# KyanChen/RSPrompter

Hardware: NVIDIA H100
Metric: images/sec (higher is better)
Workload: dtype bf16

## Files before the change

rsprompter_b200/csrc/attention.cu:

```cuda
#include <cstdlib>

#include "attention.h"
#include "sm90.cuh"

namespace rsp {

constexpr float LOG2E = 1.4426950408889634f;

__device__ __forceinline__ float fast_exp2(float x) {
  float y;
  asm("ex2.approx.ftz.f32 %0, %1;" : "=f"(y) : "f"(x));
  return y;
}
__device__ __forceinline__ uint32_t pack_f16x2(float lo, float hi) {
  __half2 v = __floats2half2_rn(lo, hi);
  return *reinterpret_cast<uint32_t*>(&v);
}
__device__ __forceinline__ uint32_t bf16x2_to_f16x2(uint32_t w) {
  return pack_f16x2(__uint_as_float(w << 16), __uint_as_float(w & 0xffff0000u));
}

template <int HD, int S>
struct AttCfg {
  static constexpr int T = S * S;
  static constexpr int BM = 128;
  static constexpr int BN = 64;
  static constexpr int NQT = (T + BM - 1) / BM;
  static constexpr int NKT = (T + BN - 1) / BN;
  static constexpr int NREL = 2 * S - 1;
  static constexpr int NTAB = NREL <= 32 ? 32 : (NREL <= 64 ? 64 : 128);
  static constexpr int TAIL = HD - 64;
  static constexpr int STAGES = 4;
  static constexpr int SP = S + 4;
  __host__ __device__ static constexpr int tile_bytes(int rows) { return rows * (128 + 2 * TAIL); }
  static constexpr int STAGE_BYTES = 2 * tile_bytes(BN);
  static constexpr int smem_bytes(int qbuf) {
    return qbuf * tile_bytes(BM) + STAGES * STAGE_BYTES + 2 * tile_bytes(NTAB) + 2 * BM * SP * 4 + 8 * 64 + 1024;
  }
  static constexpr int QBUF = smem_bytes(2) <= 227 * 1024 ? 2 : 1;
  static constexpr int Q_OFF = 0;
  static constexpr int KV_OFF = Q_OFF + QBUF * tile_bytes(BM);
  static constexpr int TAB_OFF = KV_OFF + STAGES * STAGE_BYTES;
  static constexpr int BIAS_OFF = TAB_OFF + 2 * tile_bytes(NTAB);
  static constexpr int BAR_OFF = BIAS_OFF + 2 * BM * SP * 4;
  static constexpr int SMEM_BYTES = smem_bytes(QBUF);
  static constexpr int REG_PRODUCER = 40, REG_CONSUMER = 232;
  static_assert(HD == 64 || HD == 80, "head dim");
  static_assert(NREL <= 128, "table rows");
  static_assert(SMEM_BYTES <= 227 * 1024, "shared memory");
};

struct AttDev {
  __nv_bfloat16* out;
  const int* out_row_map;
  int H;
  int D;
  int n_items;
  float scale2;
};

template <int N, int TAIL>
__device__ __forceinline__ void qk_wgmma(float (&acc)[N / 2], uint32_t qa, uint32_t qtail, uint32_t b, int b_rows) {
  acc_fence(acc);
  wgmma_fence();
#pragma unroll
  for (int k = 0; k < 4; ++k)
    Wgmma<N>::template ss<0>(acc, make_gdesc(qa + 32 * k, 16, 1024), make_gdesc(b + 32 * k, 16, 1024), k);
  if constexpr (TAIL > 0)
    Wgmma<N>::template ss<0>(acc, make_gdesc_sw32(qtail, 16, 256), make_gdesc_sw32(b + b_rows * 128, 16, 256), 1);
  wgmma_commit();
  wgmma_wait<0>();
  acc_fence(acc);
}

template <int TAIL>
__device__ __forceinline__ void load_tile(uint32_t dst, int rows, const CUtensorMap* m, const CUtensorMap* mt,
                                          uint32_t bar, int col, int row, int seq) {
  tma_load_3d(dst, m, bar, col, row, seq);
  if constexpr (TAIL > 0) tma_load_3d(dst + rows * 128, mt, bar, col + 64, row, seq);
}

template <int HD, int S>
__global__ void __launch_bounds__(384, 1)
vit_attention_kernel(const __grid_constant__ CUtensorMap tm_q, const __grid_constant__ CUtensorMap tm_q_t,
                     const __grid_constant__ CUtensorMap tm_kv, const __grid_constant__ CUtensorMap tm_kv_t,
                     const __grid_constant__ CUtensorMap tm_rh, const __grid_constant__ CUtensorMap tm_rh_t,
                     const __grid_constant__ CUtensorMap tm_rw, const __grid_constant__ CUtensorMap tm_rw_t,
                     const AttDev p) {
  using C = AttCfg<HD, S>;
  constexpr int T = C::T, BM = C::BM, BN = C::BN, NKT = C::NKT, SP = C::SP, STAGES = C::STAGES, TAIL = C::TAIL;
  constexpr int QBUF = C::QBUF;
  constexpr uint32_t TILE_KV = C::tile_bytes(BN), TILE_TAB = C::tile_bytes(C::NTAB);
  extern __shared__ __align__(1024) uint8_t smem_raw[];
  uint8_t* smem = smem_raw + ((1024u - (smem_u32(smem_raw) & 1023u)) & 1023u);
  const uint32_t sbase = smem_u32(smem);
  float* relh = reinterpret_cast<float*>(smem + C::BIAS_OFF);
  float* relw = relh + BM * SP;
  uint64_t* bar_tab = reinterpret_cast<uint64_t*>(smem + C::BAR_OFF);
  uint64_t* bar_q = bar_tab + 1;
  uint64_t* bar_qe = bar_q + QBUF;
  uint64_t* bar_k = bar_qe + QBUF;
  uint64_t* bar_v = bar_k + STAGES;
  uint64_t* bar_vc = bar_v + STAGES;
  uint64_t* bar_e = bar_vc + STAGES;

  const int warp = threadIdx.x >> 5, lane = threadIdx.x & 31;
  auto decode = [&](int item, int& q0, int& head, int& seq) {
    q0 = (item % C::NQT) * BM;
    item /= C::NQT;
    head = item % p.H;
    seq = item / p.H;
  };

  if (threadIdx.x == 0) {
    tma_prefetch_desc(&tm_q);
    tma_prefetch_desc(&tm_kv);
    mbar_init(smem_u32(bar_tab), 1);
    for (int b = 0; b < QBUF; ++b) {
      mbar_init(smem_u32(&bar_q[b]), 1);
      mbar_init(smem_u32(&bar_qe[b]), 8);
    }
    for (int s = 0; s < STAGES; ++s) {
      mbar_init(smem_u32(&bar_k[s]), 1);
      mbar_init(smem_u32(&bar_v[s]), 1);
      mbar_init(smem_u32(&bar_vc[s]), 3);
      mbar_init(smem_u32(&bar_e[s]), 8);
    }
    fence_barrier_init();
  }
  __syncthreads();

  if (warp < 4) {
    setmaxnreg_dec<C::REG_PRODUCER>();
    if (warp == 0) {
      if (lane == 0) {
        const uint32_t bq = smem_u32(bar_tab);
        mbar_expect_tx(bq, 2 * TILE_TAB);
        tma_load_2d(sbase + C::TAB_OFF, &tm_rh, bq, 0, 0);
        tma_load_2d(sbase + C::TAB_OFF + TILE_TAB, &tm_rw, bq, 0, 0);
        if constexpr (TAIL > 0) {
          tma_load_2d(sbase + C::TAB_OFF + C::NTAB * 128, &tm_rh_t, bq, 64, 0);
          tma_load_2d(sbase + C::TAB_OFF + TILE_TAB + C::NTAB * 128, &tm_rw_t, bq, 64, 0);
        }
        int g = 0;
#pragma unroll 1
        for (int item = blockIdx.x, it = 0; item < p.n_items; item += gridDim.x, ++it) {
          int q0, head, seq;
          decode(item, q0, head, seq);
          const int colq = head * HD, colk = p.D + colq, colv = 2 * p.D + colq;
          const int qb = it % QBUF;
          mbar_wait(smem_u32(&bar_qe[qb]), ((it / QBUF) & 1) ^ 1);
          mbar_expect_tx(smem_u32(&bar_q[qb]), C::tile_bytes(BM));
          load_tile<TAIL>(sbase + C::Q_OFF + qb * C::tile_bytes(BM), BM, &tm_q, &tm_q_t, smem_u32(&bar_q[qb]),
                          colq, q0, seq);
#pragma unroll 1
          for (int j = 0; j < NKT; ++j, ++g) {
            const int s = g % STAGES;
            mbar_wait(smem_u32(&bar_e[s]), ((g / STAGES) & 1) ^ 1);
            const uint32_t kb = sbase + C::KV_OFF + s * C::STAGE_BYTES;
            mbar_expect_tx(smem_u32(&bar_k[s]), TILE_KV);
            load_tile<TAIL>(kb, BN, &tm_kv, &tm_kv_t, smem_u32(&bar_k[s]), colk, j * BN, seq);
            mbar_expect_tx(smem_u32(&bar_v[s]), TILE_KV);
            load_tile<TAIL>(kb + TILE_KV, BN, &tm_kv, &tm_kv_t, smem_u32(&bar_v[s]), colv, j * BN, seq);
          }
        }
      }
    } else {
      const int t = threadIdx.x - 32;
      const int n_tiles = ((p.n_items - static_cast<int>(blockIdx.x) + gridDim.x - 1) / gridDim.x) * NKT;
#pragma unroll 1
      for (int g = 0; g < n_tiles; ++g) {
        const int s = g % STAGES;
        mbar_wait(smem_u32(&bar_v[s]), (g / STAGES) & 1);
        uint4* v = reinterpret_cast<uint4*>(smem + C::KV_OFF + s * C::STAGE_BYTES + TILE_KV);
#pragma unroll 2
        for (int i = t; i < static_cast<int>(TILE_KV / 16); i += 96) {
          uint4 w = v[i];
          w.x = bf16x2_to_f16x2(w.x);
          w.y = bf16x2_to_f16x2(w.y);
          w.z = bf16x2_to_f16x2(w.z);
          w.w = bf16x2_to_f16x2(w.w);
          v[i] = w;
        }
        fence_proxy_async_smem();
        __syncwarp();
        if (lane == 0) mbar_arrive(smem_u32(&bar_vc[s]));
      }
    }
    return;
  }

  setmaxnreg_inc<C::REG_CONSUMER>();
  const int wg = (warp >> 2) - 1;
  const int r0 = wg * 64 + (warp & 3) * 16 + (lane >> 2);
  const int cq = 2 * (lane & 3);
  constexpr bool REG_W = BN % S == 0;
  constexpr int CPS = REG_W ? S / 8 : 1;
  mbar_wait(smem_u32(bar_tab), 0);
  int g = 0;
#pragma unroll 1
  for (int item = blockIdx.x, it = 0; item < p.n_items; item += gridDim.x, ++it) {
    int q0, head, seq;
    decode(item, q0, head, seq);
    const int qb = it % QBUF;
    const uint32_t qbase = sbase + C::Q_OFF + qb * C::tile_bytes(BM);
    const uint32_t qa = qbase + wg * 64 * 128;
    const uint32_t qtail = qbase + BM * 128 + wg * 64 * 32;

    mbar_wait(smem_u32(&bar_q[qb]), (it / QBUF) & 1);
    named_bar_sync(1 + wg, 128);
#pragma unroll 1
    for (int tab = 0; tab < 2; ++tab) {
      float acc[C::NTAB / 2];
      qk_wgmma<C::NTAB, TAIL>(acc, qa, qtail, sbase + C::TAB_OFF + tab * TILE_TAB, C::NTAB);
      float* dst = tab ? relw : relh;
#pragma unroll
      for (int x = 0; x < C::NTAB / 2; ++x) {
        const int r = r0 + 8 * ((x >> 1) & 1);
        const int tq = q0 + r;
        const int qc = tab ? tq % S : tq / S;
        const int t = 8 * (x >> 2) + cq + (x & 1);
        const int k = qc + S - 1 - t;
        if (t < C::NREL && k >= 0 && k < S) dst[r * SP + k] = acc[x] * LOG2E;
      }
    }
    named_bar_sync(1 + wg, 128);

    float rw[2][2 * CPS];
    if constexpr (REG_W) {
#pragma unroll
      for (int i = 0; i < 2; ++i)
#pragma unroll
        for (int m = 0; m < 2 * CPS; ++m) rw[i][m] = relw[(r0 + 8 * i) * SP + 8 * (m >> 1) + cq + (m & 1)];
    }

    float om[32], ot[8];
#pragma unroll
    for (int y = 0; y < 32; ++y) om[y] = 0.f;
#pragma unroll
    for (int y = 0; y < 8; ++y) ot[y] = 0.f;
    float m_run[2] = {-INFINITY, -INFINITY}, l_run[2] = {0.f, 0.f};
    const float scale2 = p.scale2;

#pragma unroll(REG_W ? 1 : NKT)
    for (int j = 0; j < NKT; ++j, ++g) {
      const int s = g % STAGES;
      const uint32_t ph = (g / STAGES) & 1;
      const uint32_t kb = sbase + C::KV_OFF + s * C::STAGE_BYTES, vb = kb + TILE_KV;
      mbar_wait(smem_u32(&bar_k[s]), ph);
      float sc[BN / 2];
      qk_wgmma<BN, TAIL>(sc, qa, qtail, kb, BN);
      if (j == NKT - 1) {
        __syncwarp();
        if (lane == 0) mbar_arrive(smem_u32(&bar_qe[qb]));
      }

      float mx[2] = {-INFINITY, -INFINITY};
      if constexpr (REG_W) {
        constexpr int NB = BN / S;
        float bh[2][NB];
#pragma unroll
        for (int i = 0; i < 2; ++i)
#pragma unroll
          for (int b = 0; b < NB; ++b) bh[i][b] = relh[(r0 + 8 * i) * SP + j * NB + b];
#pragma unroll
        for (int x = 0; x < BN / 2; ++x) {
          const int i = (x >> 1) & 1;
          const float t = fmaf(sc[x], scale2, bh[i][(x >> 2) / CPS] + rw[i][((x >> 2) % CPS) * 2 + (x & 1)]);
          sc[x] = t;
          mx[i] = fmaxf(mx[i], t);
        }
      } else {
#pragma unroll
        for (int x = 0; x < BN / 2; ++x) {
          const int i = (x >> 1) & 1;
          const int key = j * BN + 8 * (x >> 2) + cq + (x & 1);
          float t = -INFINITY;
          if (T % BN == 0 || key < T) {
            const int kh = key / S, kw = key - kh * S;
            const int r = r0 + 8 * i;
            t = fmaf(sc[x], scale2, relh[r * SP + kh] + relw[r * SP + kw]);
          }
          sc[x] = t;
          mx[i] = fmaxf(mx[i], t);
        }
      }
      float alpha[2];
#pragma unroll
      for (int i = 0; i < 2; ++i) {
        mx[i] = fmaxf(mx[i], __shfl_xor_sync(0xffffffffu, mx[i], 1));
        mx[i] = fmaxf(mx[i], __shfl_xor_sync(0xffffffffu, mx[i], 2));
        const float m_new = fmaxf(m_run[i], mx[i]);
        alpha[i] = fast_exp2(m_run[i] - m_new);
        m_run[i] = m_new;
        l_run[i] *= alpha[i];
      }
#pragma unroll
      for (int y = 0; y < 32; ++y) om[y] *= alpha[(y >> 1) & 1];
#pragma unroll
      for (int y = 0; y < 8; ++y) ot[y] *= alpha[(y >> 1) & 1];
      uint32_t pa[BN / 16][4];
#pragma unroll
      for (int kk = 0; kk < BN / 16; ++kk) {
#pragma unroll
        for (int h = 0; h < 4; ++h) {
          const int x = 8 * kk + 2 * h, i = h & 1;
          const float p0 = fast_exp2(sc[x] - m_run[i]), p1 = fast_exp2(sc[x + 1] - m_run[i]);
          l_run[i] += p0 + p1;
          pa[kk][h] = pack_f16x2(p0, p1);
        }
      }
      mbar_wait(smem_u32(&bar_vc[s]), ph);
      acc_fence(om);
      acc_fence(ot);
      wgmma_fence();
#pragma unroll
      for (int kk = 0; kk < BN / 16; ++kk) {
        WgmmaRsF16<64>::rs(om, pa[kk], make_gdesc(vb + kk * 2048, BN * 128, 1024));
        if constexpr (TAIL > 0) WgmmaRsF16<16>::rs(ot, pa[kk], make_gdesc_sw32(vb + BN * 128 + kk * 512, 256, 256));
      }
      wgmma_commit();
      wgmma_wait<0>();
      acc_fence(om);
      acc_fence(ot);
      __syncwarp();
      if (lane == 0) mbar_arrive(smem_u32(&bar_e[s]));
    }

#pragma unroll
    for (int i = 0; i < 2; ++i) {
      float l = l_run[i];
      l += __shfl_xor_sync(0xffffffffu, l, 1);
      l += __shfl_xor_sync(0xffffffffu, l, 2);
      const float inv = 1.0f / l;
      const int tq = q0 + r0 + 8 * i;
      if (tq >= T) continue;
      int dst = seq * T + tq;
      if (p.out_row_map) dst = __ldg(p.out_row_map + dst);
      if (dst < 0) continue;
      __nv_bfloat16* orow = p.out + static_cast<size_t>(dst) * p.D + head * HD + cq;
#pragma unroll
      for (int nb = 0; nb < 8; ++nb)
        *reinterpret_cast<uint32_t*>(orow + nb * 8) = pack_bf16x2(om[4 * nb + 2 * i] * inv, om[4 * nb + 2 * i + 1] * inv);
      if constexpr (TAIL > 0) {
#pragma unroll
        for (int nb = 0; nb < 2; ++nb)
          *reinterpret_cast<uint32_t*>(orow + 64 + nb * 8) =
              pack_bf16x2(ot[4 * nb + 2 * i] * inv, ot[4 * nb + 2 * i + 1] * inv);
      }
    }
  }
}

template <int HD, int S>
static int launch_att(const AttentionArgs& a, cudaStream_t stream) {
  using C = AttCfg<HD, S>;
  RSP_CHECK_ARG((reinterpret_cast<uintptr_t>(a.qkv) & 15) == 0 && (reinterpret_cast<uintptr_t>(a.rel_h) & 15) == 0 &&
                (reinterpret_cast<uintptr_t>(a.rel_w) & 15) == 0 && (reinterpret_cast<uintptr_t>(a.out) & 3) == 0,
                "attention: qkv / tables must be 16-byte aligned");
  AttDev p;
  p.out = static_cast<__nv_bfloat16*>(a.out);
  p.out_row_map = a.out_row_map;
  p.H = a.H; p.D = a.H * HD;
  p.scale2 = (1.0f / sqrtf(static_cast<float>(HD))) * LOG2E;
  const uint64_t ld = 3ull * p.D;
  const uint64_t qdims[3] = {ld, static_cast<uint64_t>(C::T), static_cast<uint64_t>(a.n_seq)};
  const uint64_t qstr[2] = {ld * 2, ld * 2 * C::T};
  const uint64_t tdims[2] = {static_cast<uint64_t>(HD), static_cast<uint64_t>(C::NREL)};
  const uint64_t tstr[1] = {static_cast<uint64_t>(HD) * 2};
  const uint32_t qbox[3] = {64, C::BM, 1}, qbox_t[3] = {16, C::BM, 1};
  const uint32_t kvbox[3] = {64, C::BN, 1}, kvbox_t[3] = {16, C::BN, 1};
  const uint32_t tbox[2] = {64, static_cast<uint32_t>(C::NTAB)}, tbox_t[2] = {16, static_cast<uint32_t>(C::NTAB)};
  CUtensorMap tq, tkv, th, tw, tq_t, tkv_t, th_t, tw_t;
  RSP_TRY(make_tmap_swizzled(&tq, a.qkv, 3, qdims, qstr, qbox, 0, 128));
  RSP_TRY(make_tmap_swizzled(&tkv, a.qkv, 3, qdims, qstr, kvbox, 0, 128));
  RSP_TRY(make_tmap_swizzled(&th, a.rel_h, 2, tdims, tstr, tbox, 0, 128));
  RSP_TRY(make_tmap_swizzled(&tw, a.rel_w, 2, tdims, tstr, tbox, 0, 128));
  if (C::TAIL > 0) {
    RSP_TRY(make_tmap_swizzled(&tq_t, a.qkv, 3, qdims, qstr, qbox_t, 0, 32));
    RSP_TRY(make_tmap_swizzled(&tkv_t, a.qkv, 3, qdims, qstr, kvbox_t, 0, 32));
    RSP_TRY(make_tmap_swizzled(&th_t, a.rel_h, 2, tdims, tstr, tbox_t, 0, 32));
    RSP_TRY(make_tmap_swizzled(&tw_t, a.rel_w, 2, tdims, tstr, tbox_t, 0, 32));
  } else {
    tq_t = tq; tkv_t = tkv; th_t = th; tw_t = tw;
  }
  auto kern = vit_attention_kernel<HD, S>;
  static bool attr_set_dev[kMaxDevices] = {};
  bool& attr_set = attr_set_dev[current_device()];
  if (!attr_set) {
    RSP_CHECK_CUDA(cudaFuncSetAttribute(kern, cudaFuncAttributeMaxDynamicSharedMemorySize, C::SMEM_BYTES));
    attr_set = true;
  }
  const long long items = static_cast<long long>(a.n_seq) * a.H * C::NQT;
  RSP_CHECK_ARG(items > 0 && items < (1ll << 31), "attention: %lld query tiles", items);
  p.n_items = static_cast<int>(items);
  const int grid = static_cast<int>(items < num_sms() ? items : num_sms());
  kern<<<grid, 384, C::SMEM_BYTES, stream>>>(tq, tq_t, tkv, tkv_t, th, th_t, tw, tw_t, p);
  RSP_CHECK_LAUNCH();
  return RSP_OK;
}

int vit_attention(const AttentionArgs& a, cudaStream_t stream) {
  RSP_CHECK_ARG(a.qkv && a.rel_h && a.rel_w && a.out, "attention: null pointer");
  RSP_CHECK_ARG(a.T == a.S * a.S, "attention: T=%d is not S^2 (S=%d)", a.T, a.S);
  RSP_CHECK_ARG(a.n_seq > 0 && a.H > 0, "attention: bad n_seq/H");
  if (a.S != 14 && a.S != 32 && a.S != 64)
    return vit_attention_simt(a, stream);
  if (a.hd == 64) {
    if (a.S == 64) return launch_att<64, 64>(a, stream);
    if (a.S == 32) return launch_att<64, 32>(a, stream);
    return launch_att<64, 14>(a, stream);
  }
  if (a.hd == 80) {
    if (a.S == 64) return launch_att<80, 64>(a, stream);
    if (a.S == 32) return launch_att<80, 32>(a, stream);
    return launch_att<80, 14>(a, stream);
  }
  set_last_error("attention: head dim %d unsupported (64, 80)", a.hd);
  return RSP_ERR_UNSUPPORTED;
}

__global__ void vit_attention_simt_kernel(const __nv_bfloat16* __restrict__ qkv,
                                          const __nv_bfloat16* __restrict__ rel_h,
                                          const __nv_bfloat16* __restrict__ rel_w,
                                          __nv_bfloat16* __restrict__ out, int T, int S, int H,
                                          int hd, float scale, const int* __restrict__ out_row_map) {
  const int D = H * hd;
  const int tq = blockIdx.x * blockDim.x + threadIdx.x;
  const int head = blockIdx.y;
  const int seq = blockIdx.z;
  if (tq >= T) return;
  const int qh = tq / S, qw = tq % S;
  const __nv_bfloat16* qp = qkv + (static_cast<size_t>(seq) * T + tq) * 3 * D + head * hd;
  float q[128];
  for (int d = 0; d < hd; ++d) q[d] = __bfloat162float(qp[d]);
  float rh[128], rw[128];
  for (int k = 0; k < S; ++k) {
    float ah = 0.f, aw = 0.f;
    const __nv_bfloat16* th = rel_h + static_cast<size_t>(qh - k + S - 1) * hd;
    const __nv_bfloat16* tw = rel_w + static_cast<size_t>(qw - k + S - 1) * hd;
    for (int d = 0; d < hd; ++d) {
      ah += q[d] * __bfloat162float(th[d]);
      aw += q[d] * __bfloat162float(tw[d]);
    }
    rh[k] = ah; rw[k] = aw;
  }
  float m = -INFINITY, l = 0.f;
  float o[128];
  for (int d = 0; d < hd; ++d) o[d] = 0.f;
  for (int k = 0; k < T; ++k) {
    const __nv_bfloat16* kp = qkv + (static_cast<size_t>(seq) * T + k) * 3 * D + D + head * hd;
    const __nv_bfloat16* vp = kp + D;
    float s = 0.f;
    for (int d = 0; d < hd; ++d) s += q[d] * __bfloat162float(kp[d]);
    s = s * scale + rh[k / S] + rw[k % S];
    const float mn = fmaxf(m, s);
    const float a = expf(m - mn), pe = expf(s - mn);
    l = l * a + pe;
    for (int d = 0; d < hd; ++d) o[d] = o[d] * a + pe * __bfloat162float(vp[d]);
    m = mn;
  }
  int dst = seq * T + tq;
  if (out_row_map) dst = out_row_map[dst];
  if (dst < 0) return;
  __nv_bfloat16* op = out + static_cast<size_t>(dst) * D + head * hd;
  for (int d = 0; d < hd; ++d) op[d] = __float2bfloat16_rn(o[d] / l);
}

int vit_attention_simt(const AttentionArgs& a, cudaStream_t stream) {
  RSP_CHECK_ARG(a.qkv && a.rel_h && a.rel_w && a.out, "attention_simt: null pointer");
  RSP_CHECK_ARG(a.T == a.S * a.S && a.S <= 128 && a.hd <= 128, "attention_simt: bad T/S/hd");
  dim3 block(64);
  dim3 grid((a.T + 63) / 64, a.H, a.n_seq);
  vit_attention_simt_kernel<<<grid, block, 0, stream>>>(
      static_cast<const __nv_bfloat16*>(a.qkv), static_cast<const __nv_bfloat16*>(a.rel_h),
      static_cast<const __nv_bfloat16*>(a.rel_w), static_cast<__nv_bfloat16*>(a.out), a.T, a.S, a.H,
      a.hd, 1.0f / sqrtf(static_cast<float>(a.hd)), a.out_row_map);
// ... 6 lines not shown
```

rsprompter_b200/csrc/sm90.cuh:

```cuda
#pragma once
#include <cuda.h>
#include <cuda_bf16.h>
#include <cuda_runtime.h>
#include <stdint.h>

namespace rsp {

__device__ __forceinline__ uint32_t smem_u32(const void* p) {
  return static_cast<uint32_t>(__cvta_generic_to_shared(p));
}

__device__ __forceinline__ uint32_t elect_one() {
  uint32_t pred = 0;
  asm volatile(
      "{\n"
      ".reg .b32 rx;\n"
      ".reg .pred px;\n"
      "elect.sync rx|px, 0xffffffff;\n"
      "selp.u32 %0, 1, 0, px;\n"
      "}\n"
      : "=r"(pred));
  return pred;
}

// ... 10 lines not shown
  asm volatile("mbarrier.arrive.expect_tx.shared::cta.b64 _, [%0], %1;" ::"r"(bar), "r"(bytes)
               : "memory");
}
__device__ __forceinline__ void mbar_arrive(uint32_t bar) {
  asm volatile("mbarrier.arrive.shared::cta.b64 _, [%0];" ::"r"(bar) : "memory");
}
__device__ __forceinline__ uint32_t mbar_try_wait(uint32_t bar, uint32_t parity) {
  uint32_t ok;
  asm volatile(
      "{\n"
      ".reg .pred p;\n"
      "mbarrier.try_wait.parity.shared::cta.b64 p, [%1], %2;\n"
      "selp.u32 %0, 1, 0, p;\n"
      "}\n"
      : "=r"(ok)
      : "r"(bar), "r"(parity)
      : "memory");
  return ok;
}
__device__ __forceinline__ void mbar_wait(uint32_t bar, uint32_t parity) {
  if (mbar_try_wait(bar, parity)) return;
  long long t0 = clock64();
  uint32_t spins = 0;
  while (!mbar_try_wait(bar, parity)) {
    if ((++spins & 0x3ff) == 0 && clock64() - t0 > (1ll << 31)) __trap();
  }
}

__device__ __forceinline__ void tma_prefetch_desc(const CUtensorMap* m) {
  asm volatile("prefetch.tensormap [%0];" ::"l"(m) : "memory");
}
__device__ __forceinline__ void tma_load_2d(uint32_t dst, const CUtensorMap* m, uint32_t bar,
                                            int c0, int c1) {
  asm volatile(
      "cp.async.bulk.tensor.2d.shared::cluster.global.mbarrier::complete_tx::bytes"
      " [%0], [%1, {%3, %4}], [%2];" ::"r"(dst),
      "l"(m), "r"(bar), "r"(c0), "r"(c1)
      : "memory");
}
__device__ __forceinline__ void tma_load_3d(uint32_t dst, const CUtensorMap* m, uint32_t bar,
                                            int c0, int c1, int c2) {
  asm volatile(
      "cp.async.bulk.tensor.3d.shared::cluster.global.mbarrier::complete_tx::bytes"
      " [%0], [%1, {%3, %4, %5}], [%2];" ::"r"(dst),
      "l"(m), "r"(bar), "r"(c0), "r"(c1), "r"(c2)
      : "memory");
}
__device__ __forceinline__ void tma_load_4d(uint32_t dst, const CUtensorMap* m, uint32_t bar,
                                            int c0, int c1, int c2, int c3) {
  asm volatile(
      "cp.async.bulk.tensor.4d.shared::cluster.global.mbarrier::complete_tx::bytes"
      " [%0], [%1, {%3, %4, %5, %6}], [%2];" ::"r"(dst),
      "l"(m), "r"(bar), "r"(c0), "r"(c1), "r"(c2), "r"(c3)
      : "memory");
}

__device__ __forceinline__ void tma_store_2d(const CUtensorMap* m, uint32_t src, int c0, int c1) {
  asm volatile("cp.async.bulk.tensor.2d.global.shared::cta.bulk_group [%0, {%2, %3}], [%1];" ::"l"(m), "r"(src),
               "r"(c0), "r"(c1)
               : "memory");
}
__device__ __forceinline__ void bulk_commit() { asm volatile("cp.async.bulk.commit_group;" ::: "memory"); }
__device__ __forceinline__ void bulk_wait_read0() { asm volatile("cp.async.bulk.wait_group.read 0;" ::: "memory"); }
__device__ __forceinline__ void bulk_wait0() { asm volatile("cp.async.bulk.wait_group 0;" ::: "memory"); }

__device__ __forceinline__ uint64_t make_gdesc(uint32_t saddr, uint32_t lbo_bytes, uint32_t sbo_bytes) {
  uint64_t d = 0;
  d |= static_cast<uint64_t>((saddr & 0x3ffff) >> 4);
  d |= static_cast<uint64_t>((lbo_bytes >> 4) & 0x3fff) << 16;
  d |= static_cast<uint64_t>((sbo_bytes >> 4) & 0x3fff) << 32;
  d |= 1ull << 62;
  return d;
}

__device__ __forceinline__ uint64_t make_gdesc_sw32(uint32_t saddr, uint32_t lbo_bytes, uint32_t sbo_bytes) {
  uint64_t d = 0;
  d |= static_cast<uint64_t>((saddr & 0x3ffff) >> 4);
  d |= static_cast<uint64_t>((lbo_bytes >> 4) & 0x3fff) << 16;
  d |= static_cast<uint64_t>((sbo_bytes >> 4) & 0x3fff) << 32;
  d |= 3ull << 62;
  return d;
}

__device__ __forceinline__ void wgmma_fence() { asm volatile("wgmma.fence.sync.aligned;" ::: "memory"); }
__device__ __forceinline__ void wgmma_commit() { asm volatile("wgmma.commit_group.sync.aligned;" ::: "memory"); }
template <int N>
__device__ __forceinline__ void wgmma_wait() { asm volatile("wgmma.wait_group.sync.aligned %0;" ::"n"(N) : "memory"); }
template <int R>
__device__ __forceinline__ void acc_fence(float (&d)[R]) {
#pragma unroll
  for (int i = 0; i < R; ++i) asm volatile("" : "+f"(d[i])::"memory");
}

template <int N>
struct Wgmma;
template <> struct Wgmma<32> {
  template <int TB>
  __device__ __forceinline__ static void ss(float (&d)[16], uint64_t a, uint64_t b, uint32_t acc) {
    asm volatile(
        "{\n.reg .pred p;\n"
        "setp.ne.b32 p, %18, 0;\n"
        "wgmma.mma_async.sync.aligned.m64n32k16.f32.bf16.bf16 "
        "{" 
        "%0, %1, %2, %3, %4, %5, %6, %7, %8, %9, %10, %11, %12, %13, %14, %15"
        "}, %16, %17, p, 1, 1, 0, %19;\n}\n"
        : "+f"(d[0]), "+f"(d[1]), "+f"(d[2]), "+f"(d[3]), "+f"(d[4]), "+f"(d[5]), "+f"(d[6]), "+f"(d[7]),
          "+f"(d[8]), "+f"(d[9]), "+f"(d[10]), "+f"(d[11]), "+f"(d[12]), "+f"(d[13]), "+f"(d[14]), "+f"(d[15])
        : "l"(a), "l"(b), "r"(acc), "n"(TB));
  }
};
template <> struct Wgmma<64> {
  template <int TB>
  __device__ __forceinline__ static void ss(float (&d)[32], uint64_t a, uint64_t b, uint32_t acc) {
    asm volatile(
        "{\n.reg .pred p;\n"
        "setp.ne.b32 p, %34, 0;\n"
        "wgmma.mma_async.sync.aligned.m64n64k16.f32.bf16.bf16 "
        "{" 
        "%0, %1, %2, %3, %4, %5, %6, %7, %8, %9, %10, %11, %12, %13, %14, %15, "
        "%16, %17, %18, %19, %20, %21, %22, %23, %24, %25, %26, %27, %28, %29, %30, %31"
        "}, %32, %33, p, 1, 1, 0, %35;\n}\n"
        : "+f"(d[0]), "+f"(d[1]), "+f"(d[2]), "+f"(d[3]), "+f"(d[4]), "+f"(d[5]), "+f"(d[6]), "+f"(d[7]),
          "+f"(d[8]), "+f"(d[9]), "+f"(d[10]), "+f"(d[11]), "+f"(d[12]), "+f"(d[13]), "+f"(d[14]), "+f"(d[15]),
          "+f"(d[16]), "+f"(d[17]), "+f"(d[18]), "+f"(d[19]), "+f"(d[20]), "+f"(d[21]), "+f"(d[22]), "+f"(d[23]),
          "+f"(d[24]), "+f"(d[25]), "+f"(d[26]), "+f"(d[27]), "+f"(d[28]), "+f"(d[29]), "+f"(d[30]), "+f"(d[31])
        : "l"(a), "l"(b), "r"(acc), "n"(TB));
  }
};
template <> struct Wgmma<128> {
  template <int TB>
  __device__ __forceinline__ static void ss(float (&d)[64], uint64_t a, uint64_t b, uint32_t acc) {
    asm volatile(
        "{\n.reg .pred p;\n"
        "setp.ne.b32 p, %66, 0;\n"
        "wgmma.mma_async.sync.aligned.m64n128k16.f32.bf16.bf16 "
        "{" 
        "%0, %1, %2, %3, %4, %5, %6, %7, %8, %9, %10, %11, %12, %13, %14, %15, "
        "%16, %17, %18, %19, %20, %21, %22, %23, %24, %25, %26, %27, %28, %29, %30, %31, "
        "%32, %33, %34, %35, %36, %37, %38, %39, %40, %41, %42, %43, %44, %45, %46, %47, "
        "%48, %49, %50, %51, %52, %53, %54, %55, %56, %57, %58, %59, %60, %61, %62, %63"
        "}, %64, %65, p, 1, 1, 0, %67;\n}\n"
        : "+f"(d[0]), "+f"(d[1]), "+f"(d[2]), "+f"(d[3]), "+f"(d[4]), "+f"(d[5]), "+f"(d[6]), "+f"(d[7]),
          "+f"(d[8]), "+f"(d[9]), "+f"(d[10]), "+f"(d[11]), "+f"(d[12]), "+f"(d[13]), "+f"(d[14]), "+f"(d[15]),
          "+f"(d[16]), "+f"(d[17]), "+f"(d[18]), "+f"(d[19]), "+f"(d[20]), "+f"(d[21]), "+f"(d[22]), "+f"(d[23]),
          "+f"(d[24]), "+f"(d[25]), "+f"(d[26]), "+f"(d[27]), "+f"(d[28]), "+f"(d[29]), "+f"(d[30]), "+f"(d[31]),
          "+f"(d[32]), "+f"(d[33]), "+f"(d[34]), "+f"(d[35]), "+f"(d[36]), "+f"(d[37]), "+f"(d[38]), "+f"(d[39]),
          "+f"(d[40]), "+f"(d[41]), "+f"(d[42]), "+f"(d[43]), "+f"(d[44]), "+f"(d[45]), "+f"(d[46]), "+f"(d[47]),
          "+f"(d[48]), "+f"(d[49]), "+f"(d[50]), "+f"(d[51]), "+f"(d[52]), "+f"(d[53]), "+f"(d[54]), "+f"(d[55]),
          "+f"(d[56]), "+f"(d[57]), "+f"(d[58]), "+f"(d[59]), "+f"(d[60]), "+f"(d[61]), "+f"(d[62]), "+f"(d[63])
        : "l"(a), "l"(b), "r"(acc), "n"(TB));
  }
};
template <> struct Wgmma<256> {
  template <int TB>
  __device__ __forceinline__ static void ss(float (&d)[128], uint64_t a, uint64_t b, uint32_t acc) {
    asm volatile(
        "{\n.reg .pred p;\n"
        "setp.ne.b32 p, %130, 0;\n"
        "wgmma.mma_async.sync.aligned.m64n256k16.f32.bf16.bf16 "
        "{" 
        "%0, %1, %2, %3, %4, %5, %6, %7, %8, %9, %10, %11, %12, %13, %14, %15, "
        "%16, %17, %18, %19, %20, %21, %22, %23, %24, %25, %26, %27, %28, %29, %30, %31, "
        "%32, %33, %34, %35, %36, %37, %38, %39, %40, %41, %42, %43, %44, %45, %46, %47, "
        "%48, %49, %50, %51, %52, %53, %54, %55, %56, %57, %58, %59, %60, %61, %62, %63, "
        "%64, %65, %66, %67, %68, %69, %70, %71, %72, %73, %74, %75, %76, %77, %78, %79, "
        "%80, %81, %82, %83, %84, %85, %86, %87, %88, %89, %90, %91, %92, %93, %94, %95, "
        "%96, %97, %98, %99, %100, %101, %102, %103, %104, %105, %106, %107, %108, %109, %110, %111, "
        "%112, %113, %114, %115, %116, %117, %118, %119, %120, %121, %122, %123, %124, %125, %126, %127"
        "}, %128, %129, p, 1, 1, 0, %131;\n}\n"
        : "+f"(d[0]), "+f"(d[1]), "+f"(d[2]), "+f"(d[3]), "+f"(d[4]), "+f"(d[5]), "+f"(d[6]), "+f"(d[7]),
          "+f"(d[8]), "+f"(d[9]), "+f"(d[10]), "+f"(d[11]), "+f"(d[12]), "+f"(d[13]), "+f"(d[14]), "+f"(d[15]),
          "+f"(d[16]), "+f"(d[17]), "+f"(d[18]), "+f"(d[19]), "+f"(d[20]), "+f"(d[21]), "+f"(d[22]), "+f"(d[23]),
          "+f"(d[24]), "+f"(d[25]), "+f"(d[26]), "+f"(d[27]), "+f"(d[28]), "+f"(d[29]), "+f"(d[30]), "+f"(d[31]),
          "+f"(d[32]), "+f"(d[33]), "+f"(d[34]), "+f"(d[35]), "+f"(d[36]), "+f"(d[37]), "+f"(d[38]), "+f"(d[39]),
          "+f"(d[40]), "+f"(d[41]), "+f"(d[42]), "+f"(d[43]), "+f"(d[44]), "+f"(d[45]), "+f"(d[46]), "+f"(d[47]),
          "+f"(d[48]), "+f"(d[49]), "+f"(d[50]), "+f"(d[51]), "+f"(d[52]), "+f"(d[53]), "+f"(d[54]), "+f"(d[55]),
          "+f"(d[56]), "+f"(d[57]), "+f"(d[58]), "+f"(d[59]), "+f"(d[60]), "+f"(d[61]), "+f"(d[62]), "+f"(d[63]),
          "+f"(d[64]), "+f"(d[65]), "+f"(d[66]), "+f"(d[67]), "+f"(d[68]), "+f"(d[69]), "+f"(d[70]), "+f"(d[71]),
// ... 179 lines not shown
```

Before: 61.32.

## Software-pipeline QK and PV wgmma across key tiles and trim last tile width

Restructures the attention consumer loop so the QK wgmma for the next key tile is issued alongside the PV wgmma for the current tile, and the softmax overlaps the in-flight PV. The first and last tiles are peeled out of the loop. The last tile uses a narrower N (16/32) when only a few keys remain, and a new m64n16 wgmma is added for this. Descriptor construction now uses additive advancing instead of rebuilding each descriptor. The goal is to hide tensor-core latency behind softmax math. The cost is more live registers (two score buffers plus the packed P), and the overlap is disabled on the REG_W path.

Result: no change. 61.71 (median of 6 runs) (+0.6%).

```diff
diff --git a/rsprompter_b200/csrc/attention.cu b/rsprompter_b200/csrc/attention.cu
--- a/rsprompter_b200/csrc/attention.cu
+++ b/rsprompter_b200/csrc/attention.cu
@@ -1,4 +1,5 @@
 #include <cstdlib>
+#include <type_traits>
 
 #include "attention.h"
 #include "sm90.cuh"
@@ -27,6 +28,8 @@
   static constexpr int BN = 64;
   static constexpr int NQT = (T + BM - 1) / BM;
   static constexpr int NKT = (T + BN - 1) / BN;
+  static constexpr int LAST_KEYS = T - (NKT - 1) * BN;
+  static constexpr int NLAST = LAST_KEYS <= 16 ? 16 : (LAST_KEYS <= 32 ? 32 : BN);
   static constexpr int NREL = 2 * S - 1;
   static constexpr int NTAB = NREL <= 32 ? 32 : (NREL <= 64 ? 64 : 128);
   static constexpr int TAIL = HD - 64;
@@ -47,6 +50,7 @@
   static constexpr int REG_PRODUCER = 40, REG_CONSUMER = 232;
   static_assert(HD == 64 || HD == 80, "head dim");
   static_assert(NREL <= 128, "table rows");
+  static_assert(NKT >= 2, "the key-tile pipeline peels the first and the last tile");
   static_assert(SMEM_BYTES <= 227 * 1024, "shared memory");
 };
 
@@ -60,15 +64,19 @@
 };
 
 template <int N, int TAIL>
-__device__ __forceinline__ void qk_wgmma(float (&acc)[N / 2], uint32_t qa, uint32_t qtail, uint32_t b, int b_rows) {
+__device__ __forceinline__ void qk_issue(float (&acc)[N / 2], uint32_t qa, uint32_t qtail, uint32_t b, int b_rows) {
+  const uint64_t da = make_gdesc(qa, 16, 1024), db = make_gdesc(b, 16, 1024);
   acc_fence(acc);
   wgmma_fence();
 #pragma unroll
-  for (int k = 0; k < 4; ++k)
-    Wgmma<N>::template ss<0>(acc, make_gdesc(qa + 32 * k, 16, 1024), make_gdesc(b + 32 * k, 16, 1024), k);
+  for (int k = 0; k < 4; ++k) Wgmma<N>::template ss<0>(acc, gdesc_advance(da, 32 * k), gdesc_advance(db, 32 * k), k);
   if constexpr (TAIL > 0)
     Wgmma<N>::template ss<0>(acc, make_gdesc_sw32(qtail, 16, 256), make_gdesc_sw32(b + b_rows * 128, 16, 256), 1);
   wgmma_commit();
+}
+template <int N, int TAIL>
+__device__ __forceinline__ void qk_wgmma(float (&acc)[N / 2], uint32_t qa, uint32_t qtail, uint32_t b, int b_rows) {
+  qk_issue<N, TAIL>(acc, qa, qtail, b, b_rows);
   wgmma_wait<0>();
   acc_fence(acc);
 }
@@ -89,7 +97,7 @@
                      const AttDev p) {
   using C = AttCfg<HD, S>;
   constexpr int T = C::T, BM = C::BM, BN = C::BN, NKT = C::NKT, SP = C::SP, STAGES = C::STAGES, TAIL = C::TAIL;
-  constexpr int QBUF = C::QBUF;
+  constexpr int QBUF = C::QBUF, NLAST = C::NLAST;
   constexpr uint32_t TILE_KV = C::tile_bytes(BN), TILE_TAB = C::tile_bytes(C::NTAB);
   extern __shared__ __align__(1024) uint8_t smem_raw[];
   uint8_t* smem = smem_raw + ((1024u - (smem_u32(smem_raw) & 1023u)) & 1023u);
@@ -241,20 +249,11 @@
     for (int y = 0; y < 8; ++y) ot[y] = 0.f;
     float m_run[2] = {-INFINITY, -INFINITY}, l_run[2] = {0.f, 0.f};
     const float scale2 = p.scale2;
-
-#pragma unroll(REG_W ? 1 : NKT)
-    for (int j = 0; j < NKT; ++j, ++g) {
-      const int s = g % STAGES;
-      const uint32_t ph = (g / STAGES) & 1;
-      const uint32_t kb = sbase + C::KV_OFF + s * C::STAGE_BYTES, vb = kb + TILE_KV;
-      mbar_wait(smem_u32(&bar_k[s]), ph);
-      float sc[BN / 2];
-      qk_wgmma<BN, TAIL>(sc, qa, qtail, kb, BN);
-      if (j == NKT - 1) {
-        __syncwarp();
-        if (lane == 0) mbar_arrive(smem_u32(&bar_qe[qb]));
-      }
-
+    uint32_t pa[BN / 16][4];
+    auto kv_base = [&](int t) { return sbase + C::KV_OFF + (t % STAGES) * C::STAGE_BYTES; };
+
+    auto softmax = [&](auto& sc, int j, float (&alpha)[2]) {
+      constexpr int NR = sizeof(sc) / sizeof(float);
       float mx[2] = {-INFINITY, -INFINITY};
       if constexpr (REG_W) {
         constexpr int NB = BN / S;
@@ -264,7 +263,7 @@
 #pragma unroll
           for (int b = 0; b < NB; ++b) bh[i][b] = relh[(r0 + 8 * i) * SP + j * NB + b];
 #pragma unroll
-        for (int x = 0; x < BN / 2; ++x) {
+        for (int x = 0; x < NR; ++x) {
           const int i = (x >> 1) & 1;
           const float t = fmaf(sc[x], scale2, bh[i][(x >> 2) / CPS] + rw[i][((x >> 2) % CPS) * 2 + (x & 1)]);
           sc[x] = t;
@@ -272,7 +271,7 @@
         }
       } else {
 #pragma unroll
-        for (int x = 0; x < BN / 2; ++x) {
+        for (int x = 0; x < NR; ++x) {
           const int i = (x >> 1) & 1;
           const int key = j * BN + 8 * (x >> 2) + cq + (x & 1);
           float t = -INFINITY;
@@ -285,7 +284,6 @@
           mx[i] = fmaxf(mx[i], t);
         }
       }
-      float alpha[2];
 #pragma unroll
       for (int i = 0; i < 2; ++i) {
         mx[i] = fmaxf(mx[i], __shfl_xor_sync(0xffffffffu, mx[i], 1));
@@ -296,36 +294,98 @@
         l_run[i] *= alpha[i];
       }
 #pragma unroll
-      for (int y = 0; y < 32; ++y) om[y] *= alpha[(y >> 1) & 1];
-#pragma unroll
-      for (int y = 0; y < 8; ++y) ot[y] *= alpha[(y >> 1) & 1];
-      uint32_t pa[BN / 16][4];
-#pragma unroll
-      for (int kk = 0; kk < BN / 16; ++kk) {
+      for (int kk = 0; kk < NR / 8; ++kk) {
 #pragma unroll
         for (int h = 0; h < 4; ++h) {
           const int x = 8 * kk + 2 * h, i = h & 1;
           const float p0 = fast_exp2(sc[x] - m_run[i]), p1 = fast_exp2(sc[x + 1] - m_run[i]);
           l_run[i] += p0 + p1;
-          pa[kk][h] = pack_f16x2(p0, p1);
+          sc[x] = p0;
+          sc[x + 1] = p1;
         }
       }
-      mbar_wait(smem_u32(&bar_vc[s]), ph);
+    };
+    auto rescale_pack = [&](const auto& sc, const float (&alpha)[2]) {
+      constexpr int NR = sizeof(sc) / sizeof(float);
+#pragma unroll
+      for (int y = 0; y < 32; ++y) om[y] *= alpha[(y >> 1) & 1];
+#pragma unroll
+      for (int y = 0; y < 8; ++y) ot[y] *= alpha[(y >> 1) & 1];
+#pragma unroll
+      for (int kk = 0; kk < NR / 8; ++kk)
+#pragma unroll
+        for (int h = 0; h < 4; ++h) pa[kk][h] = pack_f16x2(sc[8 * kk + 2 * h], sc[8 * kk + 2 * h + 1]);
+    };
+    auto pv_issue = [&](auto ks, int t) {
+      const uint32_t vb = kv_base(t) + TILE_KV;
+      const uint64_t dv = make_gdesc(vb, BN * 128, 1024), dt = make_gdesc_sw32(vb + BN * 128, 256, 256);
+      mbar_wait(smem_u32(&bar_vc[t % STAGES]), (t / STAGES) & 1);
       acc_fence(om);
       acc_fence(ot);
       wgmma_fence();
 #pragma unroll
-      for (int kk = 0; kk < BN / 16; ++kk) {
-        WgmmaRsF16<64>::rs(om, pa[kk], make_gdesc(vb + kk * 2048, BN * 128, 1024));
-        if constexpr (TAIL > 0) WgmmaRsF16<16>::rs(ot, pa[kk], make_gdesc_sw32(vb + BN * 128 + kk * 512, 256, 256));
+      for (int kk = 0; kk < decltype(ks)::value; ++kk) {
+        WgmmaRsF16<64>::rs(om, pa[kk], gdesc_advance(dv, kk * 2048));
+        if constexpr (TAIL > 0) WgmmaRsF16<16>::rs(ot, pa[kk], gdesc_advance(dt, kk * 512));
       }
       wgmma_commit();
-      wgmma_wait<0>();
-      acc_fence(om);
-      acc_fence(ot);
+    };
+    auto release_stage = [&](int t) {
       __syncwarp();
-      if (lane == 0) mbar_arrive(smem_u32(&bar_e[s]));
-    }
+      if (lane == 0) mbar_arrive(smem_u32(&bar_e[t % STAGES]));
+    };
+
+    constexpr bool OVERLAP = !REG_W;
+    auto step = [&](auto n_next, int j) {
+      constexpr int N = decltype(n_next)::value;
+      float sc[N / 2];
+      if constexpr (!OVERLAP) {
+        pv_issue(std::integral_constant<int, BN / 16>(), g);
+        wgmma_wait<0>();
+        acc_fence(om);
+        acc_fence(ot);
+        release_stage(g);
+      }
+      mbar_wait(smem_u32(&bar_k[(g + 1) % STAGES]), ((g + 1) / STAGES) & 1);
+      qk_issue<N, TAIL>(sc, qa, qtail, kv_base(g + 1), BN);
+      if constexpr (OVERLAP) {
+        pv_issue(std::integral_constant<int, BN / 16>(), g);
+        wgmma_wait<1>();
+      } else {
+        wgmma_wait<0>();
+      }
+      acc_fence(sc);
+      if (j + 1 == NKT - 1) {
+        __syncwarp();
+        if (lane == 0) mbar_arrive(smem_u32(&bar_qe[qb]));
+      }
+      float alpha[2];
+      softmax(sc, j + 1, alpha);
+      if constexpr (OVERLAP) {
+        wgmma_wait<0>();
+        acc_fence(om);
+        acc_fence(ot);
+        release_stage(g);
+      }
+      ++g;
+      rescale_pack(sc, alpha);
+    };
+
+    {
+      mbar_wait(smem_u32(&bar_k[g % STAGES]), (g / STAGES) & 1);
+      float sc[BN / 2], alpha[2];
+      qk_wgmma<BN, TAIL>(sc, qa, qtail, kv_base(g), BN);
+      softmax(sc, 0, alpha);
+      rescale_pack(sc, alpha);
+    }
+#pragma unroll(REG_W ? 1 : NKT)
+    for (int j = 0; j < NKT - 2; ++j) step(std::integral_constant<int, BN>(), j);
+    step(std::integral_constant<int, NLAST>(), NKT - 2);
+    pv_issue(std::integral_constant<int, NLAST / 16>(), g);
+    wgmma_wait<0>();
+    acc_fence(om);
+    acc_fence(ot);
+    release_stage(g++);
 
 #pragma unroll
     for (int i = 0; i < 2; ++i) {
diff --git a/rsprompter_b200/csrc/sm90.cuh b/rsprompter_b200/csrc/sm90.cuh
--- a/rsprompter_b200/csrc/sm90.cuh
+++ b/rsprompter_b200/csrc/sm90.cuh
@@ -116,6 +116,8 @@
   return d;
 }
 
+__device__ __forceinline__ uint64_t gdesc_advance(uint64_t desc, uint32_t bytes) { return desc + (bytes >> 4); }
+
 __device__ __forceinline__ void wgmma_fence() { asm volatile("wgmma.fence.sync.aligned;" ::: "memory"); }
 __device__ __forceinline__ void wgmma_commit() { asm volatile("wgmma.commit_group.sync.aligned;" ::: "memory"); }
 template <int N>
@@ -128,6 +130,18 @@
 
 template <int N>
 struct Wgmma;
+template <> struct Wgmma<16> {
+  template <int TB>
+  __device__ __forceinline__ static void ss(float (&d)[8], uint64_t a, uint64_t b, uint32_t acc) {
+    asm volatile(
+        "{\n.reg .pred p;\n"
+        "setp.ne.b32 p, %10, 0;\n"
+        "wgmma.mma_async.sync.aligned.m64n16k16.f32.bf16.bf16 "
+        "{%0, %1, %2, %3, %4, %5, %6, %7}, %8, %9, p, 1, 1, 0, %11;\n}\n"
+        : "+f"(d[0]), "+f"(d[1]), "+f"(d[2]), "+f"(d[3]), "+f"(d[4]), "+f"(d[5]), "+f"(d[6]), "+f"(d[7])
+        : "l"(a), "l"(b), "r"(acc), "n"(TB));
+  }
+};
 template <> struct Wgmma<32> {
   template <int TB>
   __device__ __forceinline__ static void ss(float (&d)[16], uint64_t a, uint64_t b, uint32_t acc) {
```

## Process two 64-row query slabs per warpgroup for S=14 attention, trim last key tile

Applied to the files above, without the earlier changes.

For the S=14 (windowed) attention, each consumer warpgroup now owns two 64-row query slabs (BM=256), so each K/V tile loaded into shared memory is reused by twice as many queries. The QK wgmmas for both slabs are issued back to back before waiting, which overlaps one slab's softmax with the other's matrix multiply. The last partial key tile uses a narrower wgmma (new m64n16 variant) to skip padded columns, and bias lookups use precomputed offsets with paired float2 loads. The cost is doubled accumulator register pressure and fewer work items, which can leave SMs idle.

Result: faster. 61.74 before, 63.02 after (median of 6 runs) (+2.1%).

```diff
diff --git a/rsprompter_b200/csrc/attention.cu b/rsprompter_b200/csrc/attention.cu
--- a/rsprompter_b200/csrc/attention.cu
+++ b/rsprompter_b200/csrc/attention.cu
@@ -1,4 +1,5 @@
 #include <cstdlib>
+#include <type_traits>
 
 #include "attention.h"
 #include "sm90.cuh"
@@ -23,10 +24,12 @@
 template <int HD, int S>
 struct AttCfg {
   static constexpr int T = S * S;
-  static constexpr int BM = 128;
+  static constexpr int SL = S == 14 ? 2 : 1;
+  static constexpr int BM = 128 * SL;
   static constexpr int BN = 64;
   static constexpr int NQT = (T + BM - 1) / BM;
   static constexpr int NKT = (T + BN - 1) / BN;
+  static constexpr int LAST_N = (T - (NKT - 1) * BN + 15) / 16 * 16;
   static constexpr int NREL = 2 * S - 1;
   static constexpr int NTAB = NREL <= 32 ? 32 : (NREL <= 64 ? 64 : 128);
   static constexpr int TAIL = HD - 64;
@@ -47,6 +50,7 @@
   static constexpr int REG_PRODUCER = 40, REG_CONSUMER = 232;
   static_assert(HD == 64 || HD == 80, "head dim");
   static_assert(NREL <= 128, "table rows");
+  static_assert(BM <= 256, "TMA box rows");
   static_assert(SMEM_BYTES <= 227 * 1024, "shared memory");
 };
 
@@ -60,7 +64,7 @@
 };
 
 template <int N, int TAIL>
-__device__ __forceinline__ void qk_wgmma(float (&acc)[N / 2], uint32_t qa, uint32_t qtail, uint32_t b, int b_rows) {
+__device__ __forceinline__ void qk_issue(float (&acc)[N / 2], uint32_t qa, uint32_t qtail, uint32_t b, int b_rows) {
   acc_fence(acc);
   wgmma_fence();
 #pragma unroll
@@ -69,6 +73,11 @@
   if constexpr (TAIL > 0)
     Wgmma<N>::template ss<0>(acc, make_gdesc_sw32(qtail, 16, 256), make_gdesc_sw32(b + b_rows * 128, 16, 256), 1);
   wgmma_commit();
+}
+
+template <int N, int TAIL>
+__device__ __forceinline__ void qk_wgmma(float (&acc)[N / 2], uint32_t qa, uint32_t qtail, uint32_t b, int b_rows) {
+  qk_issue<N, TAIL>(acc, qa, qtail, b, b_rows);
   wgmma_wait<0>();
   acc_fence(acc);
 }
@@ -191,11 +200,20 @@
   }
 
   setmaxnreg_inc<C::REG_CONSUMER>();
+  constexpr int SL = C::SL, LAST_N = C::LAST_N;
   const int wg = (warp >> 2) - 1;
-  const int r0 = wg * 64 + (warp & 3) * 16 + (lane >> 2);
+  const int r0 = wg * 64 * SL + (warp & 3) * 16 + (lane >> 2);
   const int cq = 2 * (lane & 3);
   constexpr bool REG_W = BN % S == 0;
   constexpr int CPS = REG_W ? S / 8 : 1;
+  static_assert(!REG_W || SL == 1, "register rel_w terms are kept for one slab");
+  constexpr int CYC = REG_W ? 1 : S / 2;
+  int boff_h[CYC], boff_w[CYC];
+#pragma unroll
+  for (int k = 0; k < CYC; ++k) {
+    boff_h[k] = r0 * SP + (8 * k + cq) / S;
+    boff_w[k] = r0 * SP + (8 * k + cq) % S;
+  }
   mbar_wait(smem_u32(bar_tab), 0);
   int g = 0;
 #pragma unroll 1
@@ -204,24 +222,27 @@
     decode(item, q0, head, seq);
     const int qb = it % QBUF;
     const uint32_t qbase = sbase + C::Q_OFF + qb * C::tile_bytes(BM);
-    const uint32_t qa = qbase + wg * 64 * 128;
-    const uint32_t qtail = qbase + BM * 128 + wg * 64 * 32;
+    auto qa = [&](int sl) { return qbase + (wg * SL + sl) * 64 * 128; };
+    auto qtail = [&](int sl) { return qbase + BM * 128 + (wg * SL + sl) * 64 * 32; };
 
     mbar_wait(smem_u32(&bar_q[qb]), (it / QBUF) & 1);
     named_bar_sync(1 + wg, 128);
+#pragma unroll
+    for (int sl = 0; sl < SL; ++sl) {
 #pragma unroll 1
-    for (int tab = 0; tab < 2; ++tab) {
-      float acc[C::NTAB / 2];
-      qk_wgmma<C::NTAB, TAIL>(acc, qa, qtail, sbase + C::TAB_OFF + tab * TILE_TAB, C::NTAB);
-      float* dst = tab ? relw : relh;
-#pragma unroll
-      for (int x = 0; x < C::NTAB / 2; ++x) {
-        const int r = r0 + 8 * ((x >> 1) & 1);
-        const int tq = q0 + r;
-        const int qc = tab ? tq % S : tq / S;
-        const int t = 8 * (x >> 2) + cq + (x & 1);
-        const int k = qc + S - 1 - t;
-        if (t < C::NREL && k >= 0 && k < S) dst[r * SP + k] = acc[x] * LOG2E;
+      for (int tab = 0; tab < 2; ++tab) {
+        float acc[C::NTAB / 2];
+        qk_wgmma<C::NTAB, TAIL>(acc, qa(sl), qtail(sl), sbase + C::TAB_OFF + tab * TILE_TAB, C::NTAB);
+        float* dst = tab ? relw : relh;
+#pragma unroll
+        for (int x = 0; x < C::NTAB / 2; ++x) {
+          const int r = r0 + 64 * sl + 8 * ((x >> 1) & 1);
+          const int tq = q0 + r;
+          const int qc = tab ? tq % S : tq / S;
+          const int t = 8 * (x >> 2) + cq + (x & 1);
+          const int k = qc + S - 1 - t;
+          if (t < C::NREL && k >= 0 && k < S) dst[r * SP + k] = acc[x] * LOG2E;
+        }
       }
     }
     named_bar_sync(1 + wg, 128);
@@ -234,119 +255,156 @@
         for (int m = 0; m < 2 * CPS; ++m) rw[i][m] = relw[(r0 + 8 * i) * SP + 8 * (m >> 1) + cq + (m & 1)];
     }
 
-    float om[32], ot[8];
-#pragma unroll
-    for (int y = 0; y < 32; ++y) om[y] = 0.f;
-#pragma unroll
-    for (int y = 0; y < 8; ++y) ot[y] = 0.f;
-    float m_run[2] = {-INFINITY, -INFINITY}, l_run[2] = {0.f, 0.f};
+    float om[SL][32], ot[SL][8];
+    float m_run[SL][2], l_run[SL][2];
+#pragma unroll
+    for (int sl = 0; sl < SL; ++sl) {
+#pragma unroll
+      for (int y = 0; y < 32; ++y) om[sl][y] = 0.f;
+#pragma unroll
+      for (int y = 0; y < 8; ++y) ot[sl][y] = 0.f;
+#pragma unroll
+      for (int i = 0; i < 2; ++i) {
+        m_run[sl][i] = -INFINITY;
+        l_run[sl][i] = 0.f;
+      }
+    }
     const float scale2 = p.scale2;
 
-#pragma unroll(REG_W ? 1 : NKT)
-    for (int j = 0; j < NKT; ++j, ++g) {
+    auto key_tile = [&](auto n_keys, const int j) {
+      constexpr int N = decltype(n_keys)::value;
       const int s = g % STAGES;
       const uint32_t ph = (g / STAGES) & 1;
       const uint32_t kb = sbase + C::KV_OFF + s * C::STAGE_BYTES, vb = kb + TILE_KV;
       mbar_wait(smem_u32(&bar_k[s]), ph);
-      float sc[BN / 2];
-      qk_wgmma<BN, TAIL>(sc, qa, qtail, kb, BN);
-      if (j == NKT - 1) {
-        __syncwarp();
-        if (lane == 0) mbar_arrive(smem_u32(&bar_qe[qb]));
-      }
-
-      float mx[2] = {-INFINITY, -INFINITY};
-      if constexpr (REG_W) {
-        constexpr int NB = BN / S;
-        float bh[2][NB];
-#pragma unroll
-        for (int i = 0; i < 2; ++i)
-#pragma unroll
-          for (int b = 0; b < NB; ++b) bh[i][b] = relh[(r0 + 8 * i) * SP + j * NB + b];
-#pragma unroll
-        for (int x = 0; x < BN / 2; ++x) {
-          const int i = (x >> 1) & 1;
-          const float t = fmaf(sc[x], scale2, bh[i][(x >> 2) / CPS] + rw[i][((x >> 2) % CPS) * 2 + (x & 1)]);
-          sc[x] = t;
-          mx[i] = fmaxf(mx[i], t);
-        }
-      } else {
-#pragma unroll
-        for (int x = 0; x < BN / 2; ++x) {
-          const int i = (x >> 1) & 1;
-          const int key = j * BN + 8 * (x >> 2) + cq + (x & 1);
-          float t = -INFINITY;
-          if (T % BN == 0 || key < T) {
-            const int kh = key / S, kw = key - kh * S;
-            const int r = r0 + 8 * i;
-            t = fmaf(sc[x], scale2, relh[r * SP + kh] + relw[r * SP + kw]);
+      float sc[SL][N / 2];
+#pragma unroll
+      for (int sl = 0; sl < SL; ++sl) qk_issue<N, TAIL>(sc[sl], qa(sl), qtail(sl), kb, BN);
+#pragma unroll
+      for (int sl = 0; sl < SL; ++sl) {
+        wgmma_wait<SL - 1>();
+        acc_fence(sc[sl]);
+        if (sl == SL - 1 && j == NKT - 1) {
+          __syncwarp();
+          if (lane == 0) mbar_arrive(smem_u32(&bar_qe[qb]));
+        }
+
+        float mx[2] = {-INFINITY, -INFINITY};
+        if constexpr (REG_W) {
+          constexpr int NB = BN / S;
+          float bh[2][NB];
+#pragma unroll
+          for (int i = 0; i < 2; ++i)
+#pragma unroll
+            for (int b = 0; b < NB; ++b) bh[i][b] = relh[(r0 + 8 * i) * SP + j * NB + b];
+#pragma unroll
+          for (int x = 0; x < N / 2; ++x) {
+            const int i = (x >> 1) & 1;
+            const float t = fmaf(sc[sl][x], scale2, bh[i][(x >> 2) / CPS] + rw[i][((x >> 2) % CPS) * 2 + (x & 1)]);
+            sc[sl][x] = t;
+            mx[i] = fmaxf(mx[i], t);
           }
-          sc[x] = t;
-          mx[i] = fmaxf(mx[i], t);
-        }
-      }
-      float alpha[2];
-#pragma unroll
-      for (int i = 0; i < 2; ++i) {
-        mx[i] = fmaxf(mx[i], __shfl_xor_sync(0xffffffffu, mx[i], 1));
-        mx[i] = fmaxf(mx[i], __shfl_xor_sync(0xffffffffu, mx[i], 2));
-        const float m_new = fmaxf(m_run[i], mx[i]);
-        alpha[i] = fast_exp2(m_run[i] - m_new);
-        m_run[i] = m_new;
-        l_run[i] *= alpha[i];
-      }
-#pragma unroll
-      for (int y = 0; y < 32; ++y) om[y] *= alpha[(y >> 1) & 1];
-#pragma unroll
-      for (int y = 0; y < 8; ++y) ot[y] *= alpha[(y >> 1) & 1];
-      uint32_t pa[BN / 16][4];
-#pragma unroll
-      for (int kk = 0; kk < BN / 16; ++kk) {
-#pragma unroll
-        for (int h = 0; h < 4; ++h) {
-          const int x = 8 * kk + 2 * h, i = h & 1;
-          const float p0 = fast_exp2(sc[x] - m_run[i]), p1 = fast_exp2(sc[x + 1] - m_run[i]);
-          l_run[i] += p0 + p1;
-          pa[kk][h] = pack_f16x2(p0, p1);
-        }
-      }
-      mbar_wait(smem_u32(&bar_vc[s]), ph);
-      acc_fence(om);
-      acc_fence(ot);
-      wgmma_fence();
-#pragma unroll
-      for (int kk = 0; kk < BN / 16; ++kk) {
-        WgmmaRsF16<64>::rs(om, pa[kk], make_gdesc(vb + kk * 2048, BN * 128, 1024));
-        if constexpr (TAIL > 0) WgmmaRsF16<16>::rs(ot, pa[kk], make_gdesc_sw32(vb + BN * 128 + kk * 512, 256, 256));
-      }
-      wgmma_commit();
+        } else {
+          static_assert(S % 2 == 0 && SP % 2 == 0 && T % 2 == 0, "paired bias loads");
+#pragma unroll
+          for (int x = 0; x < N / 2; x += 2) {
+            const int i = (x >> 1) & 1;
+            const int m = j * (BN / 8) + (x >> 2), key = 8 * m + cq;
+            float t0 = -INFINITY, t1 = -INFINITY;
+            if (T % BN == 0 || key < T) {
+              const int rr = (64 * sl + 8 * i) * SP;
+              const float bh = relh[boff_h[m % CYC] + rr + 4 * (m / CYC)];
+              const float2 bw = *reinterpret_cast<const float2*>(relw + boff_w[m % CYC] + rr);
+              t0 = fmaf(sc[sl][x], scale2, bh + bw.x);
+              t1 = fmaf(sc[sl][x + 1], scale2, bh + bw.y);
+            }
+            sc[sl][x] = t0;
+            sc[sl][x + 1] = t1;
+            mx[i] = fmaxf(fmaxf(mx[i], t0), t1);
+          }
+        }
+        float alpha[2];
+#pragma unroll
+        for (int i = 0; i < 2; ++i) {
+          mx[i] = fmaxf(mx[i], __shfl_xor_sync(0xffffffffu, mx[i], 1));
+          mx[i] = fmaxf(mx[i], __shfl_xor_sync(0xffffffffu, mx[i], 2));
+          const float m_new = fmaxf(m_run[sl][i], mx[i]);
+          alpha[i] = fast_exp2(m_run[sl][i] - m_new);
+          m_run[sl][i] = m_new;
+          l_run[sl][i] *= alpha[i];
+        }
+#pragma unroll
+        for (int y = 0; y < 32; ++y) om[sl][y] *= alpha[(y >> 1) & 1];
+#pragma unroll
+        for (int y = 0; y < 8; ++y) ot[sl][y] *= alpha[(y >> 1) & 1];
+        uint32_t pa[N / 16][4];
+#pragma unroll
+        for (int kk = 0; kk < N / 16; ++kk) {
+#pragma unroll
+          for (int h = 0; h < 4; ++h) {
+            const int x = 8 * kk + 2 * h, i = h & 1;
+            const float p0 = fast_exp2(sc[sl][x] - m_run[sl][i]), p1 = fast_exp2(sc[sl][x + 1] - m_run[sl][i]);
+            l_run[sl][i] += p0 + p1;
+            pa[kk][h] = pack_f16x2(p0, p1);
+          }
+        }
+        if (sl == 0) mbar_wait(smem_u32(&bar_vc[s]), ph);
+        acc_fence(om[sl]);
+        acc_fence(ot[sl]);
+        wgmma_fence();
+#pragma unroll
+        for (int kk = 0; kk < N / 16; ++kk) {
+          WgmmaRsF16<64>::rs(om[sl], pa[kk], make_gdesc(vb + kk * 2048, BN * 128, 1024));
+          if constexpr (TAIL > 0)
+            WgmmaRsF16<16>::rs(ot[sl], pa[kk], make_gdesc_sw32(vb + BN * 128 + kk * 512, 256, 256));
+        }
+        wgmma_commit();
+      }
       wgmma_wait<0>();
-      acc_fence(om);
-      acc_fence(ot);
+#pragma unroll
+      for (int sl = 0; sl < SL; ++sl) {
+        acc_fence(om[sl]);
+        acc_fence(ot[sl]);
+      }
       __syncwarp();
       if (lane == 0) mbar_arrive(smem_u32(&bar_e[s]));
-    }
-
-#pragma unroll
-    for (int i = 0; i < 2; ++i) {
-      float l = l_run[i];
-      l += __shfl_xor_sync(0xffffffffu, l, 1);
-      l += __shfl_xor_sync(0xffffffffu, l, 2);
-      const float inv = 1.0f / l;
-      const int tq = q0 + r0 + 8 * i;
-      if (tq >= T) continue;
-      int dst = seq * T + tq;
-      if (p.out_row_map) dst = __ldg(p.out_row_map + dst);
-      if (dst < 0) continue;
-      __nv_bfloat16* orow = p.out + static_cast<size_t>(dst) * p.D + head * HD + cq;
-#pragma unroll
-      for (int nb = 0; nb < 8; ++nb)
-        *reinterpret_cast<uint32_t*>(orow + nb * 8) = pack_bf16x2(om[4 * nb + 2 * i] * inv, om[4 * nb + 2 * i + 1] * inv);
-      if constexpr (TAIL > 0) {
-#pragma unroll
-        for (int nb = 0; nb < 2; ++nb)
-          *reinterpret_cast<uint32_t*>(orow + 64 + nb * 8) =
-              pack_bf16x2(ot[4 * nb + 2 * i] * inv, ot[4 * nb + 2 * i + 1] * inv);
+    };
+
+#pragma unroll(REG_W ? 1 : NKT)
+    for (int j = 0; j < NKT; ++j, ++g) {
+      if constexpr (LAST_N < BN) {
+        if (j == NKT - 1) {
+          key_tile(std::integral_constant<int, LAST_N>(), j);
+          continue;
+        }
+      }
+      key_tile(std::integral_constant<int, BN>(), j);
+    }
+
+#pragma unroll
+    for (int sl = 0; sl < SL; ++sl) {
+#pragma unroll
+      for (int i = 0; i < 2; ++i) {
+        float l = l_run[sl][i];
+        l += __shfl_xor_sync(0xffffffffu, l, 1);
+        l += __shfl_xor_sync(0xffffffffu, l, 2);
+        const float inv = 1.0f / l;
+        const int tq = q0 + r0 + 64 * sl + 8 * i;
+        if (tq >= T) continue;
+        int dst = seq * T + tq;
+        if (p.out_row_map) dst = __ldg(p.out_row_map + dst);
+        if (dst < 0) continue;
+        __nv_bfloat16* orow = p.out + static_cast<size_t>(dst) * p.D + head * HD + cq;
+#pragma unroll
+        for (int nb = 0; nb < 8; ++nb)
+          *reinterpret_cast<uint32_t*>(orow + nb * 8) =
+              pack_bf16x2(om[sl][4 * nb + 2 * i] * inv, om[sl][4 * nb + 2 * i + 1] * inv);
+        if constexpr (TAIL > 0) {
+#pragma unroll
+          for (int nb = 0; nb < 2; ++nb)
+            *reinterpret_cast<uint32_t*>(orow + 64 + nb * 8) =
+                pack_bf16x2(ot[sl][4 * nb + 2 * i] * inv, ot[sl][4 * nb + 2 * i + 1] * inv);
+        }
       }
     }
   }
@@ -392,7 +450,7 @@
     attr_set = true;
   }
   const long long items = static_cast<long long>(a.n_seq) * a.H * C::NQT;
-  RSP_CHECK_ARG(items > 0 && items < (1ll << 31), "attention: %lld query tiles", items);
+  RSP_CHECK_ARG(items > 0 && items < (1ll << 31), "attention: %lld work items", items);
   p.n_items = static_cast<int>(items);
   const int grid = static_cast<int>(items < num_sms() ? items : num_sms());
   kern<<<grid, 384, C::SMEM_BYTES, stream>>>(tq, tq_t, tkv, tkv_t, th, th_t, tw, tw_t, p);
diff --git a/rsprompter_b200/csrc/sm90.cuh b/rsprompter_b200/csrc/sm90.cuh
--- a/rsprompter_b200/csrc/sm90.cuh
+++ b/rsprompter_b200/csrc/sm90.cuh
@@ -128,6 +128,18 @@
 
 template <int N>
 struct Wgmma;
+template <> struct Wgmma<16> {
+  template <int TB>
+  __device__ __forceinline__ static void ss(float (&d)[8], uint64_t a, uint64_t b, uint32_t acc) {
+    asm volatile(
+        "{\n.reg .pred p;\n"
+        "setp.ne.b32 p, %10, 0;\n"
+        "wgmma.mma_async.sync.aligned.m64n16k16.f32.bf16.bf16 "
+        "{%0, %1, %2, %3, %4, %5, %6, %7}, %8, %9, p, 1, 1, 0, %11;\n}\n"
+        : "+f"(d[0]), "+f"(d[1]), "+f"(d[2]), "+f"(d[3]), "+f"(d[4]), "+f"(d[5]), "+f"(d[6]), "+f"(d[7])
+        : "l"(a), "l"(b), "r"(acc), "n"(TB));
+  }
+};
 template <> struct Wgmma<32> {
   template <int TB>
   __device__ __forceinline__ static void ss(float (&d)[16], uint64_t a, uint64_t b, uint32_t acc) {
```
